# tenstack/batch-scheduler

Measured on AMD Instinct MI355X. Metric: pod x node fit evals/sec, higher is better.
Workload: dtype int64; 1 GPU; cfg3/tail: 10000 pods / 2000 groups / 5000 nodes, 5 int64 lanes (cpu, mem, eph, pods, gpu), seed 20260921; stages=prefilter+filter+tally+ready, parallelism=single GPU

## Files before the change

batch-scheduler_amd/csrc/bs_fast.hpp:

```cpp
#pragma once

#include "bs_kernels.hpp"
#include "bs_filter_t.hpp"

#ifdef BS_NT_TABLES
#define BS_TBL_STORE(p, v) __builtin_nontemporal_store((v), (p))
#else
#define BS_TBL_STORE(p, v) (*(p) = (v))
#endif
namespace bs {

template <bool INL = false>
__device__ __forceinline__ void arm_tally(const GroupsDev& gr, const BatchDev& b, const BatchParams& prm, uint32_t i, uint32_t nthreads);

__device__ __forceinline__ const uint8_t* range_glocal(const BatchDev& b) { return reinterpret_cast<const uint8_t*>(b.pod_ranges); }
__device__ __forceinline__ const uint32_t* range_start(const BatchDev& b, uint32_t G) { return b.pod_ranges + (G + 3u) / 4u; }
__device__ __forceinline__ const uint32_t* range_lfirst(const BatchDev& b, uint32_t G, uint32_t pod_blocks) { return range_start(b, G) + pod_blocks + 1u; }
__device__ __forceinline__ bool range_local_on(const BatchDev& b, const BatchParams& prm) {
  return b.pod_ranges && prm.do_tally && prm.do_ready && !prm.filter_deny;
}

#if BS_EMIT_MAIN
__global__ void k_pods_prep(unsigned long long* tables, uint32_t ntab, uint32_t* gstat, uint32_t ngstat, uint32_t* kcount, uint32_t* gcount, uint32_t G) {
  const uint32_t t = blockIdx.x * blockDim.x + threadIdx.x, nt = gridDim.x * blockDim.x;
// ... 263 lines not shown
    for (uint32_t j = 0; j < BS_MAX_LANES; ++j)
      if (j < sh.L()) times.v[j] = wmul(lp.mr.v[j], not_finished);
    times.present = lp.mr.present;
    res_add(out, times, sh, gate);
  }
  if (out.v[BS_LANE_PODS] == 0) out.v[BS_LANE_PODS] = mm + 1;
}
template <int TS>
__device__ __forceinline__ uint32_t filter_slot_values(const Res& cur_in, const LeaderPre& lp, Shape<TS> sh, uint32_t gate, int64_t (&R)[4], int64_t (&M)[4]) {
  Res ms, cur = cur_in;
  res_zero(ms, sh);
  res_add(ms, lp.mr, sh, gate);
  res_add(cur, ms, sh, gate);
  uint32_t ff = 0;
#pragma unroll
  for (uint32_t s = 0; s < BS_MAX_SCALARS; ++s) {
    if (s < sh.S()) {
      if ((cur.present & (1u << s)) && cur.v[4 + s] != 0) ff |= 1u;
      if ((ms.present & (1u << s)) && ms.v[4 + s] != 0) ff |= 2u;
    }
  }
#pragma unroll
  for (int j = 0; j < 4; ++j) { R[j] = cur.v[j]; M[j] = ms.v[j]; }
  return ff;
}
template <int TS, bool PUB = false>
__device__ __forceinline__ void filter_slot_from(const BatchDev& b, const BatchParams& prm, const Res& cur_in, const LeaderPre& lp, Shape<TS> sh, uint32_t gate,
                                                 uint32_t slot, bool zero_feas = true) {
  if (!lp.have_mr) return;
  int64_t R[4], M[4];
  const uint32_t ff = filter_slot_values(cur_in, lp, sh, gate, R, M);
  if (zero_feas) st_pub<PUB>(&b.fu_feas[slot], 0u);
  int64_t* dst2 = b.uparams + (size_t)slot * 8;
#pragma unroll
  for (int j = 0; j < 4; ++j) { st_pub<PUB>(&dst2[j], R[j]); st_pub<PUB>(&dst2[4 + j], M[j]); }
  st_pub<PUB>(&b.uflags[slot], ff | ((uint32_t)BS_FL_EVALUATED << 8) | (prm.stamp << 16));
}
template <int TS>
__device__ __forceinline__ uint32_t class_scan_query(const Res& cur, const LeaderPre& lp0, Shape<TS> sh, uint32_t gate, Res& q) {
  pre_allocated_from(lp0, sh, gate, q);
  res_add(q, cur, sh, gate);
  uint32_t absok = 0;
#pragma unroll
  for (uint32_t s2 = 0; s2 < BS_MAX_SCALARS; ++s2) {
    if (s2 < sh.S()) {
      const bool pres = q.present & (1u << s2);
      if (!pres || q.v[4 + s2] == 0) absok |= 1u << s2;
      if (!pres) q.v[4 + s2] = INT64_MIN;
    }
  }
  return q.present | (absok << 16);
}

template <int TS, bool PUB = false, bool SLOTS = true, bool INL = false>
__device__ __forceinline__ void fast_query_thread(const PodsDev& pods, const GroupsDev& gr, const BatchDev& b, const BatchParams& prm, uint32_t i,
                                                  uint32_t nthreads, uint32_t end = BS_INF, uint32_t t = BS_INF) {
  const Shape<TS> sh(prm.S);
  const bool valid = i < pods.p && i < end;
  const uint32_t gate = prm.eph_gate;
  const uint32_t ii = valid ? i : 0u;
  const int32_t leader0 = b.leader_epoch[0];
  const uint8_t panic0 = b.panic_epoch[0];
  const uint32_t K = prm.run_filter ? (prm.k_host ? prm.k_host : *b.kclass) : 0u;
  const int32_t gi = pods.p ? pods.group[ii] : BS_POD_NOT_GROUPED;
  const uint8_t pfl = pods.p ? pods.flags[ii] : (uint8_t)0;
  const uint64_t own = pods.p ? pods.owner[ii] : 0ull;
  const uint32_t pc = pods.p ? b.pclass[ii] : 0u;
  const uint32_t pp = pods.p ? b.ppair[ii] : BS_INF;
  Res cur;
  if (pods.p) pod_require(pods, ii, sh, gate, cur); else res_zero(cur, sh);
  arm_tally<INL>(gr, b, prm, t == BS_INF ? i : t, nthreads);
  if (i < 8 && prm.collect_stats) b.stats[i] = 0;
  const bool grouped = valid && gi >= 0 && (uint32_t)gi < gr.g;
  const uint32_t g = grouped ? (uint32_t)gi : 0u;
  const uint8_t gfl = gr.g ? gr.flags[g] : (uint8_t)0;
  const uint64_t occ0 = gr.g ? gr.occupied[g] : 0ull;
  const uint32_t fo = gr.g ? b.first_owner_s[g] : BS_INF;
  const uint32_t anchor = grouped ? b.first_pod_s[g] : i;
  LeaderPre lp0{}, lp1{};
  const bool two = prm.run_filter && prm.sop_leader0 >= 0 && prm.sop_leader0 != leader0;
  if (gr.g) {
    leader_pre_load(gr, leader0, sh, lp0);
    if (two) leader_pre_load(gr, prm.sop_leader0, sh, lp1); else lp1 = lp0;
  }
  const bool need_fo = grouped && occ0 == 0 && fo != BS_INF && i > fo;
  const uint64_t occ_fo = need_fo ? pods.owner[fo] : 0ull;
  const uint32_t owner_rank = valid ? owner_rank_of(b, prm, anchor, pods.p) : 0u;

  uint8_t code = BS_PF_PASS_NOT_GROUPED, st = 0;
  bool has_q = false;
  Res q;
  res_zero(q, sh);
  if (valid) {
    if (owner_rank == prm.rank) st |= ST_OWNED;
    if (gi == BS_POD_NOT_GROUPED) code = BS_PF_PASS_NOT_GROUPED;
    else if (pfl & BS_POD_LAST_PERMITTED) code = BS_PF_PASS_LAST_PERMITTED;
    else if (!grouped) code = BS_PF_ERR_PG_NOT_FOUND;
    else if ((gfl & BS_GROUP_DENIED) || fd_denied(b, (uint32_t)gi, i)) code = BS_PF_ERR_DENIED;
    else {
      st |= ST_ELIG;
      bool occ_err = false;
      if (occ0 != 0) occ_err = (own == 0) || (own != occ0);
      else if (need_fo) occ_err = (own == 0) || (own != occ_fo);
      if (occ_err) code = BS_PF_ERR_OCCUPIED;
      else if (panic0) code = BS_PF_PANIC_DIV0;
      else {
        st |= ST_REACH6;
        if (leader0 < 0) code = BS_PF_PASS_NO_MAX;
        else if (leader0 == gi) code = BS_PF_PASS_IS_MAX;
        else {
          pre_allocated_from(lp0, sh, gate, q);
          res_add(q, cur, sh, gate);
          code = BS_PF_PASS_RESERVE_FITS;
          has_q = (st & ST_OWNED) != 0;
        }
      }
    }
    if (has_q) st |= ST_QUERY;
    b.tcode[i] = code;
    b.stage[i] = st;
  }
  BS_STAMP(1, 1);
  {
    __shared__ uint32_t s_reach;
    if (threadIdx.x == 0) s_reach = BS_INF;
    __syncthreads();
    const unsigned long long rb = __ballot(valid && (st & ST_REACH6));
    if (rb && lane_id() == __ffsll((long long)rb) - 1) atomicMin(&s_reach, i);
    __syncthreads();
    if (threadIdx.x == 0) st_pub<INL>(&b.first_reach64[blockIdx.x], ((unsigned long long)prm.seq_inv << 32) | s_reach);
  }
  BS_STAMP(1, 2);
  const uint32_t qslot = has_q ? pc : 0u;
  bool fill = SLOTS && wave_elect_by_key(qslot, has_q);
  bool w1 = false, w2 = false;
  if (SLOTS && prm.run_filter) {
    const bool may = valid && (st & ST_OWNED) && BS_PF_IS_PASS(code) && grouped;
    w1 = wave_elect_by_key(pc, may && leader0 >= 0 && leader0 != gi);
    w2 = wave_elect_by_key(pc, may && prm.sop_leader0 >= 0 && prm.sop_leader0 != gi);
  }
  if constexpr (PUB) {
    uint32_t o1 = 0, o2 = 0, o3 = 0;
    if (w1) o1 = __hip_atomic_exchange(&b.uclaim[pc], prm.stamp, __ATOMIC_RELAXED, __HIP_MEMORY_SCOPE_AGENT);
    if (w2) o2 = __hip_atomic_exchange(&b.uclaim[pc + K], prm.stamp, __ATOMIC_RELAXED, __HIP_MEMORY_SCOPE_AGENT);
    if (fill) o3 = __hip_atomic_exchange(&b.qstamp_s[qslot], prm.stamp, __ATOMIC_RELAXED, __HIP_MEMORY_SCOPE_AGENT);
    if (w1 && o1 == prm.stamp) w1 = false;
    if (w2 && o2 == prm.stamp) w2 = false;
    if (fill && o3 == prm.stamp) fill = false;
  }
  if (w1) filter_slot_from<TS, PUB>(b, prm, cur, lp0, sh, gate, pc);
  if (w2) filter_slot_from<TS, PUB>(b, prm, cur, lp1, sh, gate, pc + K);
  BS_STAMP(1, 3);
  if (has_q) {
    b.qpos[i] = qslot;
    atomicMin(&b.pair_firstq[pp], ((unsigned long long)prm.seq_inv << 32) | i);
  }
  if (fill) {
    uint32_t absok = 0;
#pragma unroll
    for (uint32_t s = 0; s < BS_MAX_SCALARS; ++s) {
      if (s < sh.S()) {
        const bool pres = q.present & (1u << s);
        if (!pres || q.v[4 + s] == 0) absok |= 1u << s;
        if (!pres) q.v[4 + s] = INT64_MIN;
      }
    }
    const uint32_t slot = qslot;
    int64_t* dst = b.qreq_s + (size_t)slot * prm.LP;
#pragma unroll
    for (uint32_t j = 0; j < BS_MAX_LANES; ++j)
      if (j < prm.LP) st_pub<PUB>(&dst[j], j < sh.L() ? q.v[j] : (int64_t)INT64_MIN);
    st_pub<PUB>(&b.qflags_s[slot], q.present | (absok << 16));
    st_pub<PUB>(&b.qtab_s[slot], (int32_t)0);
    st_pub<PUB>(&b.first_row[slot], BS_INF);
// ... 32 lines not shown
    Res ms;
    res_zero(ms, sh);
    if (have && lp.have_mr) res_add(ms, lp.mr, sh, gate);
    uint32_t ff = (have && lp.have_mr) ? 1u : 0u;
#pragma unroll
    for (uint32_t q = 0; q < BS_MAX_SCALARS; ++q)
      if (q < sh.S() && (ms.present & (1u << q)) && ms.v[4 + q] != 0) ff |= 2u;
    const unsigned long long holds = __ballot(l[0] >= ms.v[0] && l[1] >= ms.v[1] && l[2] >= ms.v[2] && l[3] >= ms.v[3]);
    if (stores) {
      b.nodew[nodew_pair(stride, s, w)] = ok;
      b.nodew[nodew_pair(stride, s, w) + 1] = ~holds;
    }
    if (blk == 0 && threadIdx.x == 0) {
#pragma unroll
      for (int j = 0; j < 4; ++j) b.nodew[nodew_ref_lane(stride, s, j)] = (uint64_t)ms.v[j];
      b.nodew[nodew_ref_flags(stride, s)] = ff;
    }
  }
}

template <int TS>
__global__ __launch_bounds__(kTblChunk) void k_fast_query_tables(PodsDev pods, GroupsDev gr, NodesDev nd, BatchDev b, BatchDev bt, BatchParams prm,
                                                                 const TableDesc* forced, uint32_t nchunks, uint32_t query_blocks) {
  BS_STAMP(1, 0);
  if (blockIdx.x < query_blocks) fast_query_thread<TS>(pods, gr, b, prm, blockIdx.x * kTblChunk + threadIdx.x, query_blocks * kTblChunk);
  else if (blockIdx.x < query_blocks + nchunks) tables_local_fast<TS>(nd, bt, prm, forced, blockIdx.x - query_blocks);
  else node_words_block<TS>(gr, nd, b, prm, blockIdx.x - query_blocks - nchunks);
  BS_STAMP(1, 7);
}

template <int NL>
__device__ __forceinline__ unsigned long long rows_cover(unsigned long long m, const int64_t (&a)[BS_MAX_LANES], const int64_t (&r)[BS_MAX_LANES]) {
  asm volatile("s_mov_b64 exec, %[m]\n\tv_cmpx_ge_i64 vcc, %[a0], %[r0]\n\tv_cmpx_ge_i64 vcc, %[a1], %[r1]\n\tv_cmpx_ge_i64 vcc, %[a2], %[r2]\n\t"
               "v_cmpx_ge_i64 vcc, %[a3], %[r3]\n\ts_mov_b64 %[m], exec\n\ts_mov_b64 exec, -1"
               : [m] "+s"(m)
               : [a0] "v"(a[0]), [r0] "v"(r[0]), [a1] "v"(a[1]), [r1] "v"(r[1]), [a2] "v"(a[2]), [r2] "v"(r[2]), [a3] "v"(a[3]), [r3] "v"(r[3])
               : "vcc");
#pragma unroll
  for (int j = 4; j < NL; ++j)
    asm volatile("s_mov_b64 exec, %[m]\n\tv_cmpx_ge_i64 vcc, %[a], %[r]\n\ts_mov_b64 %[m], exec\n\ts_mov_b64 exec, -1" : [m] "+s"(m) : [a] "v"(a[j]), [r] "v"(r[j]) : "vcc");
  return m;
}
#ifndef BS_SCAN_BALLOT
#define BS_SCAN_BALLOT 1
#endif
constexpr uint32_t kSpinBound = 1u << 18;
__device__ __forceinline__ void test_chaos_delay() {
#ifdef BS_TEST_CHAOS
  uint32_t h = (blockIdx.x + 1u) * 2654435761u ^ (uint32_t)wall_clock64() * 40503u;
  h ^= h >> 15; h *= 2246822519u; h ^= h >> 13;
  for (uint32_t s = 0; s < (h & 15u); ++s) __builtin_amdgcn_s_sleep(127);
#endif
}
constexpr uint32_t kStepSlotsMax = 256;
__device__ __forceinline__ bool step_wait(const uint32_t* word, uint32_t base, uint32_t need, int32_t* h_err) {
  uint32_t spins = 0;
  while ((uint32_t)(ld_agent(word) - base) < need) {
    __builtin_amdgcn_s_sleep(1);
    if (++spins > kSpinBound) { if (h_err) __hip_atomic_store(h_err, 1, __ATOMIC_RELAXED, __HIP_MEMORY_SCOPE_SYSTEM); return false; }
  }
  return true;
}
constexpr uint32_t kScanRecChunks = 64;
constexpr uint32_t kFeasRecGroups = 32;
#ifndef BS_GATHER_DIRECT
#define BS_GATHER_DIRECT 8
#endif
constexpr uint32_t kGatherDirectBlocks = BS_GATHER_DIRECT;
constexpr uint32_t kRecStride = 32;
constexpr uint32_t kTkSlots = 32, kTkTab = 48, kTkP1 = 64, kTkDone = 64 + 16 * 16, kTkWays = 16, kTkWords = 64 + 2 * 16 * 16;
__device__ __forceinline__ void spread_add(uint32_t* words, uint32_t who) {
  (void)__hip_atomic_fetch_add(&words[16u * (who % kTkWays)], 1u, __ATOMIC_RELAXED, __HIP_MEMORY_SCOPE_AGENT);
}
__device__ __forceinline__ bool spread_wait(const uint32_t* words, uint32_t base, uint32_t need, int32_t* h_err) {
  uint32_t spins = 0;
  for (;;) {
    uint32_t v = lane_id() < (int)kTkWays ? ld_agent(&words[16u * (uint32_t)lane_id()]) : 0u;
#pragma unroll
    for (int o = 1; o < (int)kTkWays; o <<= 1) v += (uint32_t)__shfl_xor((int)v, o);
    v = (uint32_t)__builtin_amdgcn_readfirstlane((int)v);
    if ((uint32_t)(v - base) >= need) return true;
    __builtin_amdgcn_s_sleep(4);
    if (++spins > kSpinBound) { if (h_err && lane_id() == 0) __hip_atomic_store(h_err, 1, __ATOMIC_RELAXED, __HIP_MEMORY_SCOPE_SYSTEM); return false; }
  }
}
template <int TS, bool REGS = false>
__device__ __forceinline__ void table_scan_block(const NodesDev& nd, const BatchDev& b, const BatchParams& prm, const TableDesc* forced, uint32_t chunk, uint32_t nchunks,
                                                 uint32_t share, uint32_t nshares, uint32_t pod_blocks, uint32_t tk_pods0, uint32_t tk_tab0, const GroupsDev& gr,
                                                 const int64_t* ckeys, const uint32_t* cpres, uint32_t kcap, bool direct = false, uint32_t forced_cls = 0) {
  __shared__ unsigned long long s_wtot[BS_MAX_LANES][4];
  __shared__ uint32_t s_kp[BS_MAX_SCALARS];
  __shared__ unsigned long long s_off[BS_MAX_LANES];
  __shared__ uint32_t s_kpg[BS_MAX_SCALARS];
  __shared__ int64_t s_req[kStepSlotsMax][BS_MAX_LANES];
  __shared__ uint32_t s_qf[kStepSlotsMax];
  __shared__ uint32_t s_first[kStepSlotsMax];
  BS_STAMP(2, 0);
  const Shape<TS> sh(prm.S);
  const uint32_t L = sh.L(), S = sh.S(), LP = prm.LP;
  const uint32_t k = chunk * kTblChunk + threadIdx.x;
  const bool in_range = REGS ? k < nd.n : k < nd.m;
  const uint32_t n = REGS ? (in_range ? k : 0u) : (in_range ? nd.kmap[k] : 0u);
  const TableDesc d = REGS ? TableDesc{forced_cls, 0.7f} : *forced;
  const uint32_t fw = nd.fit[(size_t)d.cls * nd.fit_words + (n >> 5)];
  const uint8_t fl = nd.flags[n];
  const bool valid = in_range && (!REGS || !(fl & BS_NODE_SKIP_MASK));
  const uint32_t ap = nd.apres[n], rp = nd.rpres[n];
  int64_t al[BS_MAX_LANES], rq[BS_MAX_LANES];
#pragma unroll
  for (uint32_t j = 0; j < BS_MAX_LANES; ++j) {
    if (j < L) {
      al[j] = nd.alloc[(size_t)j * nd.stride + n];
      rq[j] = nd.req[(size_t)j * nd.stride + n];
    }
  }
  const uint32_t K = prm.k_host ? prm.k_host : *b.kclass;
  const uint32_t per = (K + nshares - 1u) / nshares, s_lo = share * per, s_hi = min(K, s_lo + per);
  Res raw;
  int32_t leader0 = -1;
  uint8_t panic0 = 0;
  LeaderPre lp0{};
  if constexpr (REGS) {
    const uint32_t cc = s_lo + threadIdx.x < s_hi ? s_lo + threadIdx.x : 0u;
#pragma unroll
    for (uint32_t j = 0; j < BS_MAX_LANES; ++j)
      if (j < L) raw.v[j] = ckeys[(size_t)j * kcap + cc];
    raw.present = cpres[cc];
    leader0 = b.leader_epoch[0];
    panic0 = b.panic_epoch[0];
    if (gr.g) leader_pre_load(gr, leader0, sh, lp0);
  }
  const bool fit = valid && ((fw >> (n & 31u)) & 1u) && !(fl & BS_NODE_TAINT_ERR);
  const uint32_t pres = fit ? (ap & rp) : 0u;
  if (threadIdx.x < BS_MAX_SCALARS) s_kp[threadIdx.x] = BS_INF;
  for (uint32_t t = threadIdx.x; t < kStepSlotsMax; t += kTblChunk) s_first[t] = BS_INF;
  unsigned long long incl[BS_MAX_LANES];
  const int w = wave_id();
#pragma unroll
  for (uint32_t j = 0; j < BS_MAX_LANES; ++j) {
    incl[j] = 0;
    if (j < L) {
      const bool live = fit && (j < 4 || (pres & (1u << (j - 4)))) && !(j == BS_LANE_EPH && !prm.eph_gate);
      const unsigned long long left = live ? (unsigned long long)wsub(scale_f32(al[j], d.pct), rq[j]) : 0ull;
      incl[j] = wave_incl_scan_add_u64(left);
      if (lane_id() == 63) s_wtot[j][w] = incl[j];
    }
  }
  __syncthreads();
#pragma unroll
// ... 365 lines not shown
  if (threadIdx.x == 0) {
    __hip_atomic_store(&b.ticket[0], 0u, __ATOMIC_RELAXED, __HIP_MEMORY_SCOPE_AGENT);
    if constexpr (WT && BS_HOME_WT) __hip_atomic_store(b.h_tag, prm.host_tag, __ATOMIC_RELAXED, __HIP_MEMORY_SCOPE_SYSTEM);
    else __hip_atomic_store(b.h_tag, prm.host_tag, __ATOMIC_RELEASE, __HIP_MEMORY_SCOPE_SYSTEM);
  }
}

__device__ __forceinline__ void tally_quorum_atomic(const BatchDev& b, const BatchParams& prm, bool grouped, uint32_t g, bool admit, uint32_t want, uint32_t ma,
                                                    uint32_t need) {
  unsigned long long mine = 0;
  bool asked = false;
  unsigned long long todo = __ballot(grouped);
  const unsigned long long adm = __ballot(grouped && admit);
  for (int round = 0; todo && round < kElectRounds; ++round) {
    const int leader = __ffsll((long long)todo) - 1;
    const uint32_t k0 = (uint32_t)__builtin_amdgcn_readlane((int)g, leader);
    const unsigned long long same = __ballot(grouped && g == k0) & todo;
    if (lane_id() == leader) {
      mine = ((unsigned long long)__popcll(same) << 32) | (unsigned long long)__popcll(same & adm);
      asked = true;
    }
    todo &= ~same;
  }
  if (todo & (1ull << lane_id())) {
    mine = (1ull << 32) | (admit ? 1ull : 0ull);
    asked = true;
  }
  unsigned long long got = 0;
  if (asked) got = __hip_atomic_fetch_add(&b.admit64[g], mine, __ATOMIC_RELAXED, __HIP_MEMORY_SCOPE_AGENT);
  if (asked) {
    const unsigned long long tot = got + mine;
    if ((uint32_t)(tot >> 32) == want) {
      const uint32_t ad = (uint32_t)tot;
      const uint8_t rd = (ma + ad) >= need ? 1 : 0;
      b.admit[g] = ad;
      b.ready[g] = rd;
      if (prm.host_tag) { st_home(&b.h_admit[g], ad); st_home(&b.h_ready[g], rd); }
    }
  }
}
template <bool WT = false>
__device__ __forceinline__ void tally_tail(const GroupsDev& gr, const BatchDev& b, const BatchParams& prm, bool grouped, uint32_t g, bool admit,
                                           uint32_t nblocks) {
  if (prm.do_tally && prm.do_ready) {
    uint32_t want = 0, ma = 0, mm = 0, sc = 0;
    if (grouped) { want = b.gcount[g]; ma = gr.matched[g]; mm = gr.min_member[g]; sc = gr.status_scheduled[g]; }
    tally_quorum_atomic(b, prm, grouped, g, admit, want, ma, (uint32_t)(mm - sc));
  } else if (prm.do_tally) {
    wave_aggregated_add(b.admit, g, grouped && admit);
  }
  final_tail<WT>(b, prm, nblocks);
}

constexpr uint32_t kLocalTag = 0x80000000u;
template <bool WT = false>
__device__ __forceinline__ void tally_tail_whole(const GroupsDev& gr, const BatchDev& b, const BatchParams& prm, bool grouped, uint32_t g, bool admit,
                                                 uint32_t nblocks, uint32_t gwant, uint32_t ma, uint32_t need, uint32_t* s_adm) {
  if (prm.do_tally && prm.do_ready) {
    const bool local = grouped && (gwant & kLocalTag);
    const uint32_t lslot = gwant & 0xFFu;
    if (local && admit) atomicAdd(&s_adm[lslot], 1u);
    __syncthreads();
    if (local && lslot == threadIdx.x) {
      const uint32_t ad = s_adm[lslot];
      const uint8_t rd = (ma + ad) >= need ? 1 : 0;
      b.admit[g] = ad;
      b.ready[g] = rd;
      if (prm.host_tag) { st_home(&b.h_admit[g], ad); st_home(&b.h_ready[g], rd); }
    }
    tally_quorum_atomic(b, prm, grouped && !local, g, admit, gwant, ma, need);
  } else if (prm.do_tally) {
    wave_aggregated_add(b.admit, g, grouped && admit);
  }
  final_tail<WT>(b, prm, nblocks);
}


template <bool INL = false>
__device__ __forceinline__ void fast_final_block(const PodsDev& pods, const GroupsDev& gr, const NodesDev& nd, const BatchDev& b, const BatchParams& prm,
                                                 uint32_t query_blocks, uint32_t bx, uint32_t nblocks, uint32_t producers, uint32_t tk_p1 = 0, uint32_t aux = 0,
                                                 uint32_t tk_done = 0, uint32_t hint_blocks = 0, uint32_t p0 = BS_INF, uint32_t p1 = BS_INF) {
  __shared__ uint32_t s_first_reach;
  __shared__ uint32_t s_rowk[INL ? kStepSlotsMax : 1u], s_feask[INL ? 2u * kStepSlotsMax : 1u], s_ladm[INL ? 256u : 1u], s_gw[INL ? 3u : 1u][INL ? 256u : 1u];
  BS_STAMP(3, 0);
  if constexpr (INL) {
    s_ladm[threadIdx.x] = 0u;
    if (threadIdx.x < 64) (void)spread_wait(&b.ticket[kTkP1], tk_p1, query_blocks, b.h_err);
    __syncthreads();
  }
  const uint32_t dx = bx * 256u + threadIdx.x;
  const uint32_t i = p0 == BS_INF ? dx : p0 + threadIdx.x;
  const bool valid = i < pods.p && (p0 == BS_INF || i < p1);
  uint8_t code0 = 0, st0 = 0;
  int32_t gi0 = BS_POD_NOT_GROUPED;
  uint32_t qpos0 = 0, pclass0 = 0, pair0 = BS_INF;
  uint32_t lfirst = BS_INF;
  if (valid) { code0 = b.tcode[i]; st0 = b.stage[i]; gi0 = pods.group[i]; qpos0 = b.qpos[i]; pclass0 = b.pclass[i]; pair0 = b.ppair[i]; }
  if (INL && valid && range_local_on(b, prm)) lfirst = range_lfirst(b, gr.g, query_blocks)[i];
  const uint32_t K = prm.k_host ? prm.k_host : *b.kclass;
  const int32_t leader_now = b.leader_epoch[0];
  if (threadIdx.x < 64) {
    uint32_t found = BS_INF;
    for (uint32_t b0 = 0; b0 < query_blocks && found == BS_INF; b0 += 64u) {
      const uint32_t bk = b0 + threadIdx.x;
      uint32_t v = BS_INF;
      if (bk < query_blocks) {
        const unsigned long long w = INL ? ld_agent64(&b.first_reach64[bk]) : b.first_reach64[bk];
        if ((uint32_t)(w >> 32) == prm.seq_inv) v = (uint32_t)w;
      }
      const unsigned long long any = __ballot(v != BS_INF);
      if (any) found = (uint32_t)__shfl((int)v, __ffsll((long long)any) - 1);
    }
    if (threadIdx.x == 0) s_first_reach = found;
  }
  const bool owned = valid && (st0 & ST_OWNED);
  const bool walk = owned && (st0 & ST_ELIG);
  const bool grouped = valid && gi0 >= 0 && (uint32_t)gi0 < gr.g;
  uint32_t row_q = BS_INF, row_c = BS_INF, feas0 = 0, feas1 = 0;
  unsigned long long head = ~0ull, own_fq = ~0ull, own_next = ~0ull;
  if (walk) {
    head = b.pair_head[gi0];
    if (pair0 != BS_INF) { own_fq = INL ? ld_agent64(&b.pair_firstq[pair0]) : b.pair_firstq[pair0]; own_next = b.pair_next[pair0]; }
  }
  if constexpr (INL) {
    if (prm.do_tally && prm.do_ready) {
      uint32_t gwant = 0, gma = 0, gneed = 0;
      if (grouped) {
        gma = gr.matched[gi0];
        gneed = (uint32_t)(gr.min_member[gi0] - gr.status_scheduled[gi0]);
        gwant = lfirst != BS_INF ? kLocalTag | (lfirst - p0) : b.gcount[gi0];
      }
      s_gw[0][threadIdx.x] = gwant;
      s_gw[1][threadIdx.x] = gma;
      s_gw[2][threadIdx.x] = gneed;
    }
  }
  if (producers) {
    asm volatile("s_waitcnt vmcnt(0)" ::: "memory");
    if constexpr (INL) {
      const uint32_t tagw = prm.seq_inv, U = prm.run_filter ? 2u * K : 0u;
      uint32_t groups = 0;
      if (prm.run_filter) {
        uint32_t tiles, bpw, nchunk;
        step_filter_split(K, (nd.n + 63u) / 64u, aux, tiles, bpw, nchunk);
        groups = (nchunk + 3u) / 4u;
      }
      const unsigned long long none = ((unsigned long long)tagw << 32) | BS_INF, zero = (unsigned long long)tagw << 32;
      BS_STAMP(3, 4);
      if (query_blocks > kGatherDirectBlocks) {
        if (threadIdx.x < 64) (void)spread_wait(&b.ticket[kTkDone], tk_done, hint_blocks, b.h_err);
      } else
      for (uint32_t spins = 0;; ++spins) {
        uint32_t andt = tagw, ort = tagw, row = BS_INF, fs[2] = {0u, 0u};
        if (threadIdx.x < K) {
          const unsigned long long* rec = b.scan_rec + threadIdx.x;
          for (uint32_t c0 = 0; c0 < producers; c0 += 8u) {
            unsigned long long w[8];
#pragma unroll
            for (uint32_t u = 0; u < 8u; ++u) w[u] = c0 + u < producers ? ld_agent64(&rec[(size_t)(c0 + u) * kStepSlotsMax]) : none;
#pragma unroll
            for (uint32_t u = 0; u < 8u; ++u) { andt &= (uint32_t)(w[u] >> 32); ort |= (uint32_t)(w[u] >> 32); row = min(row, (uint32_t)w[u]); }
          }
        }
#pragma unroll
        for (uint32_t h = 0; h < 2u; ++h) {
          const uint32_t slot = threadIdx.x + 256u * h;
          if (slot < U) {
            const unsigned long long* rec = b.feas_rec + slot;
            for (uint32_t g0 = 0; g0 < groups; g0 += 8u) {
              unsigned long long w[8];
#pragma unroll
              for (uint32_t u = 0; u < 8u; ++u) w[u] = g0 + u < groups ? ld_agent64(&rec[(size_t)(g0 + u) * (2u * kStepSlotsMax)]) : zero;
#pragma unroll
              for (uint32_t u = 0; u < 8u; ++u) { andt &= (uint32_t)(w[u] >> 32); ort |= (uint32_t)(w[u] >> 32); fs[h] += (uint32_t)w[u]; }
            }
          }
        }
        const bool timed_out = spins > kSpinBound / 2u;
        if (__syncthreads_and((andt == tagw && ort == tagw) || timed_out)) {
          if (threadIdx.x < K) s_rowk[threadIdx.x] = row;
#pragma unroll
          for (uint32_t h = 0; h < 2u; ++h)
            if (threadIdx.x + 256u * h < U) s_feask[threadIdx.x + 256u * h] = fs[h];
          if (timed_out && threadIdx.x == 0 && b.h_err) __hip_atomic_store(b.h_err, 1, __ATOMIC_RELAXED, __HIP_MEMORY_SCOPE_SYSTEM);
          BS_COUNT(3, 5, spins + 1u);
          break;
        }
        __builtin_amdgcn_s_sleep(2);
// ... 45 lines not shown
          }
        }
        denied = fr < i;
        if (prm.commit && fr == i) b.fast_reject[gi] = fr;
      }
      if (denied) code = BS_PF_ERR_DENIED;
      else if (st & ST_QUERY) {
        if (row_q == BS_INF) { code = BS_PF_REJECT_RESERVE; fk = BS_K_NONE; }
        else fk = INL ? row_q : nd.kmap[row_q];
      }
    } else {
      code = BS_PF_NOT_OWNED;
    }
    b.pf_code[i] = code;
    b.pf_first_k[i] = fk;
    const bool reached = i >= first_reach;
    const int32_t leader = reached ? leader_now : prm.sop_leader0;
    b.pf_leader[i] = leader;
    if (prm.host_tag) { st_home(&b.h_pf_code[i], code); st_home(&b.h_pf_first_k[i], fk); st_home(&b.h_pf_leader[i], leader); }
    const bool pass = code != BS_PF_NOT_OWNED && BS_PF_IS_PASS(code);
    uint32_t feasible = 1u, slot = 0;
    uint8_t fl = BS_FL_NOT_RUN;
    if (prm.run_filter) {
      if (pass) {
        if (gi == BS_POD_NOT_GROUPED) fl = BS_FL_PASS_NOT_GROUPED;
        else if (gi < 0 || (uint32_t)gi >= gr.g) fl = BS_FL_ERR_PG_NOT_FOUND;
        else if (leader < 0) fl = BS_FL_PANIC_NIL_MAX;
        else if (leader == gi) fl = BS_FL_PASS_IS_MAX;
        else { fl = BS_FL_EVALUATED; slot = pclass0 + (reached ? 0u : K); }
      }
      feasible = fl == BS_FL_EVALUATED ? (reached ? feas0 : feas1) : (fl < 16u ? nd.n : 0u);
      b.fu_slot[i] = slot;
      b.fl_feasible[i] = feasible;
    } else {
      b.fl_feasible[i] = 0;
    }
    b.fl_code[i] = fl;
    b.fflags[i] = (uint32_t)fl << 8;
    if (prm.host_tag) { st_home(&b.h_fl_code[i], fl); st_home(&b.h_fl_feasible[i], prm.run_filter ? feasible : 0u); st_home(&b.h_fl_slot[i], slot); }
    if (gi >= 0 && (uint32_t)gi < gr.g && pass && feasible > 0) admit = true;
    if (prm.filter_deny && fl == BS_FL_EVALUATED && feasible < nd.n) atomicMin(&b.fd_event[gi], ((unsigned long long)prm.seq_inv << 32) | i);
  }
  if (gathered) {
    if (prm.run_filter)
      for (uint32_t k = dx; k < 2u * K; k += nblocks * 256u) b.fu_feas[k] = s_feask[INL ? k : 0u];
  }
  if (prm.host_tag && prm.run_filter) {
    const uint32_t U = min(2u * K, b.hstride);
    for (uint32_t k = dx; k < U; k += nblocks * 256u) st_home(&b.h_feas[k], gathered ? s_feask[INL ? k : 0u] : ld_agent(&b.fu_feas[k]));
  }
  BS_STAMP(3, 2);
  if (!prm.filter_deny) {
    if constexpr (INL)
      tally_tail_whole<true>(gr, b, prm, grouped, grouped ? (uint32_t)gi0 : 0u, admit, nblocks, s_gw[0][threadIdx.x], s_gw[1][threadIdx.x], s_gw[2][threadIdx.x], s_ladm);
    else
      tally_tail<true>(gr, b, prm, grouped, grouped ? (uint32_t)gi0 : 0u, admit, nblocks);
  }
  BS_STAMP(3, 7);
}

template <int S>
__global__ __launch_bounds__(256) void k_fast_scan_filter(PodsDev pods, NodesDev nd, BatchDev bt, BatchParams prm, uint32_t m, uint32_t jcap,
                                                          uint32_t scan_blocks, uint32_t filter_waves, uint32_t ustride) {
  __shared__ int64_t s_rows[4][64][4 + S];
  if (blockIdx.x < scan_blocks)
    scan_loop<S, true, 1>(bt, prm, m, jcap, 0u, 0u, 1u, blockIdx.x, scan_blocks, s_rows[wave_id()]);
  else
    filter_loop<2>(pods, nd, bt, filter_waves, 1u, ustride, prm.collect_stats, blockIdx.x - scan_blocks, gridDim.x - scan_blocks, prm.stamp, 2u * prm.k_host);
}
template <int S>
__global__ __launch_bounds__(256) void k_fast_scan(BatchDev bt, BatchParams prm, uint32_t m, uint32_t jcap) {
  __shared__ int64_t s_rows[4][64][4 + S];
  scan_loop<S, true, 1>(bt, prm, m, jcap, 0u, 0u, 1u, blockIdx.x, gridDim.x, s_rows[wave_id()]);
}
template <int PU, bool DB>
__global__ __launch_bounds__(256) void k_fast_filter(PodsDev pods, NodesDev nd, BatchDev bt, BatchParams prm, uint32_t filter_waves, uint32_t ustride) {
  filter_loop<2, PU, DB>(pods, nd, bt, filter_waves, 1u, ustride, prm.collect_stats, blockIdx.x, gridDim.x, prm.stamp, 2u * prm.k_host);
}
#if BS_EMIT_FAST
__global__ __launch_bounds__(256) __attribute__((amdgpu_waves_per_eu(7))) void k_fast_filter_w7(PodsDev pods, NodesDev nd, BatchDev bt, BatchParams prm, uint32_t filter_waves,
                                                                                                uint32_t ustride) {
  filter_loop<2, 2, false>(pods, nd, bt, filter_waves, 1u, ustride, prm.collect_stats, blockIdx.x, gridDim.x, prm.stamp, 2u * prm.k_host);
}
#endif
#if BS_EMIT_FAST
__global__ __launch_bounds__(256) void k_fast_filter_t(NodesDev nd, BatchDev bt, BatchParams prm, uint32_t filter_waves, uint32_t ustride, uint32_t by_tile) {
  filter_loop_t<false>(nd, bt, filter_waves, ustride, prm.collect_stats, blockIdx.x, gridDim.x, prm.stamp, 2u * prm.k_host, by_tile);
}
#endif
template <int S>
__global__ __launch_bounds__(256) __attribute__((amdgpu_waves_per_eu(S <= 1 ? 4 : 1))) void k_fast_scan_filter_t(NodesDev nd, BatchDev bt, BatchParams prm, uint32_t m, uint32_t jcap, uint32_t scan_blocks,
                                                            uint32_t filter_waves, uint32_t ustride, uint32_t form) {
  __shared__ int64_t s_rows[4][64][4 + S];
  const uint32_t filter_first = form & 1u, by_tile = form & 2u;
  const uint32_t filter_blocks = gridDim.x - scan_blocks;
  const bool is_scan = filter_first ? blockIdx.x >= filter_blocks : blockIdx.x < scan_blocks;
  BS_STAMP(2, 0);
  if (is_scan)
    scan_loop<S, true, 1>(bt, prm, m, jcap, 0u, 0u, 1u, filter_first ? blockIdx.x - filter_blocks : blockIdx.x, scan_blocks, s_rows[wave_id()]);
  else
    filter_loop_t<true>(nd, bt, filter_waves, ustride, prm.collect_stats, filter_first ? blockIdx.x : blockIdx.x - scan_blocks, filter_blocks, prm.stamp, 2u * prm.k_host, by_tile);
  BS_STAMP(2, 7);
}
#if BS_EMIT_MAIN
__global__ __launch_bounds__(256) void k_fast_final(PodsDev pods, GroupsDev gr, NodesDev nd, BatchDev b, BatchParams prm, uint32_t query_blocks) {
  fast_final_block(pods, gr, nd, b, prm, query_blocks, blockIdx.x, gridDim.x, 0u);
}
#endif

template <int S>
__global__ __launch_bounds__(256) void k_fast_scan_filter_final(PodsDev pods, GroupsDev gr, NodesDev nd, BatchDev b, BatchDev bt, BatchParams prm, uint32_t m,
                                                                uint32_t jcap, uint32_t scan_blocks, uint32_t filter_blocks, uint32_t filter_waves,
                                                                uint32_t ustride, uint32_t query_blocks) {
  __shared__ int64_t s_rows[4][64][4 + S];
  const uint32_t producers = scan_blocks + filter_blocks;
  test_chaos_delay();
#ifdef BS_TEST_LATE_ROLE_B
  {
    const int role = blockIdx.x < scan_blocks ? 0 : blockIdx.x < producers ? 1 : 2;
    if (role == BS_TEST_LATE_ROLE_B) for (int spin = 0; spin < 20; ++spin) __builtin_amdgcn_s_sleep(127);
  }
#endif
  if (blockIdx.x < producers) {
    BS_STAMP(2, 0);
    if (blockIdx.x < scan_blocks)
      scan_loop<S, true, 2>(bt, prm, m, jcap, 0u, 0u, 1u, blockIdx.x, scan_blocks, s_rows[wave_id()]);
    else
      filter_loop<2>(pods, nd, bt, filter_waves, 1u, ustride, prm.collect_stats, blockIdx.x - scan_blocks, filter_blocks, prm.stamp, 2u * prm.k_host);
    asm volatile("s_waitcnt vmcnt(0)" ::: "memory");
    __syncthreads();
    if (threadIdx.x == 0) (void)__hip_atomic_fetch_add(&b.ticket[1], 1u, __ATOMIC_RELAXED, __HIP_MEMORY_SCOPE_AGENT);
    BS_STAMP(2, 7);
    return;
  }
  fast_final_block(pods, gr, nd, b, prm, query_blocks, blockIdx.x - producers, gridDim.x - producers, producers);
}

template <int TS, bool WHOLE>
__global__ __launch_bounds__(kTblChunk) void k_fast_step_a(PodsDev pods, GroupsDev gr, NodesDev nd, BatchDev b, BatchDev bt, BatchParams prm, const TableDesc* forced,
                                                           uint32_t nchunks, uint32_t query_blocks, uint32_t nshares, uint32_t filter_blocks, uint32_t filter_waves,
                                                           uint32_t ustride, uint32_t tk_pods0, uint32_t tk_tab0, uint32_t param_blocks, const int64_t* ckeys,
                                                           const uint32_t* cpres, uint32_t kcap, uint32_t tk_p1, uint32_t tk_done, uint32_t forced_cls) {
  BS_STAMP(1, 0);
  test_chaos_delay();
  const uint32_t tb = nchunks * nshares;
#ifdef BS_TEST_LATE_ROLE
  {
    const int role = blockIdx.x < query_blocks ? 0 : blockIdx.x < query_blocks + param_blocks ? 1 : blockIdx.x < query_blocks + param_blocks + tb ? 2 : 3;
    if (role == BS_TEST_LATE_ROLE) for (int spin = 0; spin < 20; ++spin) __builtin_amdgcn_s_sleep(127);
  }
#endif
  const uint32_t producers = param_blocks ? param_blocks : query_blocks;
  const bool direct = query_blocks <= kGatherDirectBlocks;
  if (blockIdx.x < query_blocks) {
    if constexpr (WHOLE) {
      const uint32_t p0 = b.pod_ranges ? range_start(b, gr.g)[blockIdx.x] : blockIdx.x * kTblChunk;
      const uint32_t p1 = b.pod_ranges ? range_start(b, gr.g)[blockIdx.x + 1u] : pods.p;
      fast_query_thread<TS, false, false, true>(pods, gr, b, prm, p0 + threadIdx.x, query_blocks * kTblChunk, p1, blockIdx.x * kTblChunk + threadIdx.x);
      asm volatile("s_waitcnt vmcnt(0)" ::: "memory");
      __syncthreads();
      if (threadIdx.x == 0) spread_add(&b.ticket[kTkP1], blockIdx.x);
      fast_final_block<true>(pods, gr, nd, b, prm, query_blocks, blockIdx.x, query_blocks, nchunks, tk_p1, filter_waves, tk_done, tb + filter_blocks, p0, p1);
    } else if (param_blocks) {
      fast_query_thread<TS, false, false>(pods, gr, b, prm, blockIdx.x * kTblChunk + threadIdx.x, query_blocks * kTblChunk);
    } else {
      fast_query_thread<TS, true>(pods, gr, b, prm, blockIdx.x * kTblChunk + threadIdx.x, query_blocks * kTblChunk);
      BS_STAMP(1, 4);
      asm volatile("s_waitcnt vmcnt(0)" ::: "memory");
      __syncthreads();
      BS_STAMP(1, 5);
      if (threadIdx.x == 0) (void)__hip_atomic_fetch_add(&b.ticket[kTkSlots], 1u, __ATOMIC_RELAXED, __HIP_MEMORY_SCOPE_AGENT);
    }
  } else if (blockIdx.x < query_blocks + param_blocks) {
    class_slots_block<TS>(gr, b, prm, ckeys, cpres, kcap, blockIdx.x - query_blocks, !(WHOLE && direct));
  } else if (blockIdx.x < query_blocks + param_blocks + tb) {
    const uint32_t x = blockIdx.x - query_blocks - param_blocks;
    table_scan_block<TS, WHOLE>(nd, bt, prm, forced, x / nshares, nchunks, x % nshares, nshares, producers, tk_pods0, tk_tab0, gr, ckeys, cpres, kcap, direct, forced_cls);
    if constexpr (WHOLE) {
      if (!direct) {
        asm volatile("s_waitcnt vmcnt(0)" ::: "memory");
        __syncthreads();
        if (threadIdx.x == 0) spread_add(&b.ticket[kTkDone], blockIdx.x);
      }
    }
  } else if constexpr (WHOLE) {
    step_filter_block<TS>(gr, nd, bt, prm, ckeys, cpres, kcap, filter_waves, ustride, blockIdx.x - query_blocks - param_blocks - tb, filter_blocks, direct, tk_pods0, producers);
    if (!direct) {
      asm volatile("s_waitcnt vmcnt(0)" ::: "memory");
      __syncthreads();
      if (threadIdx.x == 0) spread_add(&b.ticket[kTkDone], blockIdx.x);
    }
  } else {
    __shared__ uint32_t s_go;
    if (threadIdx.x == 0) {
      s_go = step_wait(&b.ticket[kTkSlots], tk_pods0, producers, b.h_err) ? 1u : 0u;
      __builtin_amdgcn_fence(__ATOMIC_ACQUIRE, "agent");
    }
    __syncthreads();
    if (!s_go) return;
    filter_loop<2>(pods, nd, bt, filter_waves, 1u, ustride, prm.collect_stats, blockIdx.x - query_blocks - param_blocks - tb, filter_blocks, prm.stamp, 2u * prm.k_host);
  }
  BS_STAMP(1, 7);
}


template <int TS>
__global__ __launch_bounds__(kTblChunk) void k_tables_local_nofix(NodesDev nd, BatchDev b, BatchParams prm, uint32_t nchunks, uint32_t cstride,
                                                                  uint32_t gstride) {
  const uint32_t slot = blockIdx.x;
  if (!b.needed[slot]) return;
  BatchDev bt = b;
  bt.tables = b.tables + (size_t)slot * prm.mcap * prm.LP;
  bt.kp = b.kp + (size_t)slot * 16;
  bt.chunk_tot = b.chunk_tot + (size_t)slot * cstride * 16;
  bt.chunk_kp = b.chunk_kp + (size_t)slot * cstride * 16;
  bt.gmax = b.gmax + (size_t)slot * gstride * prm.LP;
  const TableDesc d = table_desc(slot, prm.C, nullptr);
  tables_local_fast<TS>(nd, bt, prm, &d, blockIdx.y);
}

#if BS_EMIT_MAIN
__global__ __launch_bounds__(kLeaderBlock) void k_leader_scan(GroupsDev gr, BatchDev b) {
  __shared__ unsigned long long s_w[kLeaderBlock / 64];
  __shared__ uint32_t s_p[kLeaderBlock / 64];
  __shared__ unsigned long long s_carry;
  __shared__ uint32_t s_pcarry, s_nexact, s_exact[64];
  const uint32_t E1 = *b.nepochs;
  auto key_of = [&](uint32_t g, bool& panic) -> unsigned long long {
    if (gr.flags[g] & BS_GROUP_SCHEDULED_LATCH) return 0ull;
    const uint32_t f = leader_finished(gr, g, panic);
// ... 85 lines not shown
```

Before: 3713 billion evals/s.

## Share LDS arena across block roles and hand pod state to final block via LDS

Introduces a single shared-memory arena in the fused step kernel, used by the table-scan role and the whole-pod query/final role, so the kernel's LDS footprint is the max rather than the sum of both roles. The query phase writes per-pod code, stage, group, class and pair into LDS so the final block reads them locally instead of reloading tcode/stage/group/pclass/ppair from global memory. Group metadata (pair_head, pair_next, matched, min_member, status, gcount) loads are moved before the ticket spin-wait to overlap their latency with waiting. Risk: qpos is replaced by pclass in the inline path, and the early global loads assume the data are stable before the wait.

```diff
diff --git a/batch-scheduler_amd/csrc/bs_fast.hpp b/batch-scheduler_amd/csrc/bs_fast.hpp
--- a/batch-scheduler_amd/csrc/bs_fast.hpp
+++ b/batch-scheduler_amd/csrc/bs_fast.hpp
@@ -339,9 +339,39 @@
   return q.present | (absok << 16);
 }
 
+constexpr uint32_t kStepSlotsMax = 256;
+struct PodLds {
+  uint32_t* rowk;
+  uint32_t* feask;
+  uint32_t* ladm;
+  uint32_t* gw;
+  uint32_t* pk;
+  uint32_t* gi;
+  uint32_t* pc;
+  uint32_t* pair;
+};
+constexpr uint32_t kPodRec = 1u << 31;
+constexpr uint32_t kLocalTag = 0x80000000u;
+constexpr uint32_t kArenaTableBytes = kStepSlotsMax * BS_MAX_LANES * 8u + 2u * kStepSlotsMax * 4u;
+constexpr uint32_t kArenaPodBytes = (3u * kStepSlotsMax + 256u + 3u * 256u + 4u * 256u) * 4u;
+constexpr uint32_t kStepArenaBytes = kArenaTableBytes > kArenaPodBytes ? kArenaTableBytes : kArenaPodBytes;
+__device__ __forceinline__ PodLds pod_lds(unsigned char* arena) {
+  uint32_t* w = reinterpret_cast<uint32_t*>(arena);
+  PodLds o;
+  o.rowk = w; w += kStepSlotsMax;
+  o.feask = w; w += 2u * kStepSlotsMax;
+  o.ladm = w; w += 256u;
+  o.gw = w; w += 3u * 256u;
+  o.pk = w; w += 256u;
+  o.gi = w; w += 256u;
+  o.pc = w; w += 256u;
+  o.pair = w;
+  return o;
+}
+
 template <int TS, bool PUB = false, bool SLOTS = true, bool INL = false>
 __device__ __forceinline__ void fast_query_thread(const PodsDev& pods, const GroupsDev& gr, const BatchDev& b, const BatchParams& prm, uint32_t i,
-                                                  uint32_t nthreads, uint32_t end = BS_INF, uint32_t t = BS_INF) {
+                                                  uint32_t nthreads, uint32_t end = BS_INF, uint32_t t = BS_INF, const PodLds* pl = nullptr) {
   const Shape<TS> sh(prm.S);
   const bool valid = i < pods.p && i < end;
   const uint32_t gate = prm.eph_gate;
@@ -407,6 +437,13 @@
     b.tcode[i] = code;
     b.stage[i] = st;
   }
+  if constexpr (INL) {
+    const uint32_t x = threadIdx.x;
+    pl->pk[x] = valid ? (kPodRec | (uint32_t)code | ((uint32_t)st << 8)) : 0u;
+    pl->gi[x] = valid ? (uint32_t)gi : (uint32_t)BS_POD_NOT_GROUPED;
+    pl->pc[x] = valid ? pc : 0u;
+    pl->pair[x] = valid ? pp : BS_INF;
+  }
   BS_STAMP(1, 1);
   {
     __shared__ uint32_t s_reach;
@@ -545,7 +582,6 @@
   for (uint32_t s = 0; s < (h & 15u); ++s) __builtin_amdgcn_s_sleep(127);
 #endif
 }
-constexpr uint32_t kStepSlotsMax = 256;
 __device__ __forceinline__ bool step_wait(const uint32_t* word, uint32_t base, uint32_t need, int32_t* h_err) {
   uint32_t spins = 0;
   while ((uint32_t)(ld_agent(word) - base) < need) {
@@ -580,14 +616,15 @@
 template <int TS, bool REGS = false>
 __device__ __forceinline__ void table_scan_block(const NodesDev& nd, const BatchDev& b, const BatchParams& prm, const TableDesc* forced, uint32_t chunk, uint32_t nchunks,
                                                  uint32_t share, uint32_t nshares, uint32_t pod_blocks, uint32_t tk_pods0, uint32_t tk_tab0, const GroupsDev& gr,
-                                                 const int64_t* ckeys, const uint32_t* cpres, uint32_t kcap, bool direct = false, uint32_t forced_cls = 0) {
+                                                 const int64_t* ckeys, const uint32_t* cpres, uint32_t kcap, unsigned char* arena, bool direct = false,
+                                                 uint32_t forced_cls = 0) {
   __shared__ unsigned long long s_wtot[BS_MAX_LANES][4];
   __shared__ uint32_t s_kp[BS_MAX_SCALARS];
   __shared__ unsigned long long s_off[BS_MAX_LANES];
   __shared__ uint32_t s_kpg[BS_MAX_SCALARS];
-  __shared__ int64_t s_req[kStepSlotsMax][BS_MAX_LANES];
-  __shared__ uint32_t s_qf[kStepSlotsMax];
-  __shared__ uint32_t s_first[kStepSlotsMax];
+  int64_t (*s_req)[BS_MAX_LANES] = reinterpret_cast<int64_t (*)[BS_MAX_LANES]>(arena);
+  uint32_t* s_qf = reinterpret_cast<uint32_t*>(arena + kStepSlotsMax * BS_MAX_LANES * 8u);
+  uint32_t* s_first = s_qf + kStepSlotsMax;
   BS_STAMP(2, 0);
   const Shape<TS> sh(prm.S);
   const uint32_t L = sh.L(), S = sh.S(), LP = prm.LP;
@@ -1059,7 +1096,6 @@
   final_tail<WT>(b, prm, nblocks);
 }
 
-constexpr uint32_t kLocalTag = 0x80000000u;
 template <bool WT = false>
 __device__ __forceinline__ void tally_tail_whole(const GroupsDev& gr, const BatchDev& b, const BatchParams& prm, bool grouped, uint32_t g, bool admit,
                                                  uint32_t nblocks, uint32_t gwant, uint32_t ma, uint32_t need, uint32_t* s_adm) {
@@ -1086,24 +1122,48 @@
 template <bool INL = false>
 __device__ __forceinline__ void fast_final_block(const PodsDev& pods, const GroupsDev& gr, const NodesDev& nd, const BatchDev& b, const BatchParams& prm,
                                                  uint32_t query_blocks, uint32_t bx, uint32_t nblocks, uint32_t producers, uint32_t tk_p1 = 0, uint32_t aux = 0,
-                                                 uint32_t tk_done = 0, uint32_t hint_blocks = 0, uint32_t p0 = BS_INF, uint32_t p1 = BS_INF) {
+                                                 uint32_t tk_done = 0, uint32_t hint_blocks = 0, uint32_t p0 = BS_INF, uint32_t p1 = BS_INF,
+                                                 unsigned char* arena = nullptr) {
   __shared__ uint32_t s_first_reach;
-  __shared__ uint32_t s_rowk[INL ? kStepSlotsMax : 1u], s_feask[INL ? 2u * kStepSlotsMax : 1u], s_ladm[INL ? 256u : 1u], s_gw[INL ? 3u : 1u][INL ? 256u : 1u];
+  PodLds L{};
+  if constexpr (INL) L = pod_lds(arena);
+  uint32_t* const s_rowk = L.rowk;
+  uint32_t* const s_feask = L.feask;
+  uint32_t* const s_ladm = L.ladm;
   BS_STAMP(3, 0);
-  if constexpr (INL) {
-    s_ladm[threadIdx.x] = 0u;
-    if (threadIdx.x < 64) (void)spread_wait(&b.ticket[kTkP1], tk_p1, query_blocks, b.h_err);
-    __syncthreads();
-  }
   const uint32_t dx = bx * 256u + threadIdx.x;
   const uint32_t i = p0 == BS_INF ? dx : p0 + threadIdx.x;
   const bool valid = i < pods.p && (p0 == BS_INF || i < p1);
   uint8_t code0 = 0, st0 = 0;
   int32_t gi0 = BS_POD_NOT_GROUPED;
   uint32_t qpos0 = 0, pclass0 = 0, pair0 = BS_INF;
-  uint32_t lfirst = BS_INF;
-  if (valid) { code0 = b.tcode[i]; st0 = b.stage[i]; gi0 = pods.group[i]; qpos0 = b.qpos[i]; pclass0 = b.pclass[i]; pair0 = b.ppair[i]; }
-  if (INL && valid && range_local_on(b, prm)) lfirst = range_lfirst(b, gr.g, query_blocks)[i];
+  unsigned long long head = ~0ull, own_fq = ~0ull, own_next = ~0ull;
+  if constexpr (INL) {
+    const uint32_t x = threadIdx.x, pk = L.pk[x];
+    code0 = (uint8_t)pk;
+    st0 = (uint8_t)(pk >> 8);
+    gi0 = (int32_t)L.gi[x];
+    pclass0 = L.pc[x];
+    qpos0 = pclass0;
+    pair0 = L.pair[x];
+    const bool grp = valid && gi0 >= 0 && (uint32_t)gi0 < gr.g;
+    uint32_t lfirst = BS_INF, gwant = 0, gma = 0, gmm = 0, gsc = 0;
+    if (valid && range_local_on(b, prm)) lfirst = range_lfirst(b, gr.g, query_blocks)[i];
+    if (grp) {
+      head = b.pair_head[gi0];
+      if (pair0 != BS_INF) own_next = b.pair_next[pair0];
+      if (prm.do_tally && prm.do_ready) { gma = gr.matched[gi0]; gmm = gr.min_member[gi0]; gsc = gr.status_scheduled[gi0]; gwant = b.gcount[gi0]; }
+    }
+    s_ladm[x] = 0u;
+    if (x < 64) (void)spread_wait(&b.ticket[kTkP1], tk_p1, query_blocks, b.h_err);
+    __syncthreads();
+    if (grp && prm.do_tally && prm.do_ready && lfirst != BS_INF) gwant = kLocalTag | (lfirst - p0);
+    L.gw[x] = gwant;
+    L.gw[256u + x] = gma;
+    L.gw[512u + x] = (uint32_t)(gmm - gsc);
+  } else if (valid) {
+    code0 = b.tcode[i]; st0 = b.stage[i]; gi0 = pods.group[i]; qpos0 = b.qpos[i]; pclass0 = b.pclass[i]; pair0 = b.ppair[i];
+  }
   const uint32_t K = prm.k_host ? prm.k_host : *b.kclass;
   const int32_t leader_now = b.leader_epoch[0];
   if (threadIdx.x < 64) {
@@ -1124,23 +1184,11 @@
   const bool walk = owned && (st0 & ST_ELIG);
   const bool grouped = valid && gi0 >= 0 && (uint32_t)gi0 < gr.g;
   uint32_t row_q = BS_INF, row_c = BS_INF, feas0 = 0, feas1 = 0;
-  unsigned long long head = ~0ull, own_fq = ~0ull, own_next = ~0ull;
-  if (walk) {
+  if constexpr (INL) {
+    if (walk && pair0 != BS_INF) own_fq = ld_agent64(&b.pair_firstq[pair0]);
+  } else if (walk) {
     head = b.pair_head[gi0];
-    if (pair0 != BS_INF) { own_fq = INL ? ld_agent64(&b.pair_firstq[pair0]) : b.pair_firstq[pair0]; own_next = b.pair_next[pair0]; }
-  }
-  if constexpr (INL) {
-    if (prm.do_tally && prm.do_ready) {
-      uint32_t gwant = 0, gma = 0, gneed = 0;
-      if (grouped) {
-        gma = gr.matched[gi0];
-        gneed = (uint32_t)(gr.min_member[gi0] - gr.status_scheduled[gi0]);
-        gwant = lfirst != BS_INF ? kLocalTag | (lfirst - p0) : b.gcount[gi0];
-      }
-      s_gw[0][threadIdx.x] = gwant;
-      s_gw[1][threadIdx.x] = gma;
-      s_gw[2][threadIdx.x] = gneed;
-    }
+    if (pair0 != BS_INF) { own_fq = b.pair_firstq[pair0]; own_next = b.pair_next[pair0]; }
   }
   if (producers) {
     asm volatile("s_waitcnt vmcnt(0)" ::: "memory");
@@ -1292,7 +1340,7 @@
   BS_STAMP(3, 2);
   if (!prm.filter_deny) {
     if constexpr (INL)
-      tally_tail_whole<true>(gr, b, prm, grouped, grouped ? (uint32_t)gi0 : 0u, admit, nblocks, s_gw[0][threadIdx.x], s_gw[1][threadIdx.x], s_gw[2][threadIdx.x], s_ladm);
+      tally_tail_whole<true>(gr, b, prm, grouped, grouped ? (uint32_t)gi0 : 0u, admit, nblocks, L.gw[threadIdx.x], L.gw[256u + threadIdx.x], L.gw[512u + threadIdx.x], s_ladm);
     else
       tally_tail<true>(gr, b, prm, grouped, grouped ? (uint32_t)gi0 : 0u, admit, nblocks);
   }
@@ -1383,6 +1431,7 @@
                                                            const uint32_t* cpres, uint32_t kcap, uint32_t tk_p1, uint32_t tk_done, uint32_t forced_cls) {
   BS_STAMP(1, 0);
   test_chaos_delay();
+  __shared__ __align__(16) unsigned char s_arena[kStepArenaBytes];
   const uint32_t tb = nchunks * nshares;
 #ifdef BS_TEST_LATE_ROLE
   {
@@ -1396,11 +1445,12 @@
     if constexpr (WHOLE) {
       const uint32_t p0 = b.pod_ranges ? range_start(b, gr.g)[blockIdx.x] : blockIdx.x * kTblChunk;
       const uint32_t p1 = b.pod_ranges ? range_start(b, gr.g)[blockIdx.x + 1u] : pods.p;
-      fast_query_thread<TS, false, false, true>(pods, gr, b, prm, p0 + threadIdx.x, query_blocks * kTblChunk, p1, blockIdx.x * kTblChunk + threadIdx.x);
+      const PodLds pl = pod_lds(s_arena);
+      fast_query_thread<TS, false, false, true>(pods, gr, b, prm, p0 + threadIdx.x, query_blocks * kTblChunk, p1, blockIdx.x * kTblChunk + threadIdx.x, &pl);
       asm volatile("s_waitcnt vmcnt(0)" ::: "memory");
       __syncthreads();
       if (threadIdx.x == 0) spread_add(&b.ticket[kTkP1], blockIdx.x);
-      fast_final_block<true>(pods, gr, nd, b, prm, query_blocks, blockIdx.x, query_blocks, nchunks, tk_p1, filter_waves, tk_done, tb + filter_blocks, p0, p1);
+      fast_final_block<true>(pods, gr, nd, b, prm, query_blocks, blockIdx.x, query_blocks, nchunks, tk_p1, filter_waves, tk_done, tb + filter_blocks, p0, p1, s_arena);
     } else if (param_blocks) {
       fast_query_thread<TS, false, false>(pods, gr, b, prm, blockIdx.x * kTblChunk + threadIdx.x, query_blocks * kTblChunk);
     } else {
@@ -1415,7 +1465,8 @@
     class_slots_block<TS>(gr, b, prm, ckeys, cpres, kcap, blockIdx.x - query_blocks, !(WHOLE && direct));
   } else if (blockIdx.x < query_blocks + param_blocks + tb) {
     const uint32_t x = blockIdx.x - query_blocks - param_blocks;
-    table_scan_block<TS, WHOLE>(nd, bt, prm, forced, x / nshares, nchunks, x % nshares, nshares, producers, tk_pods0, tk_tab0, gr, ckeys, cpres, kcap, direct, forced_cls);
+    table_scan_block<TS, WHOLE>(nd, bt, prm, forced, x / nshares, nchunks, x % nshares, nshares, producers, tk_pods0, tk_tab0, gr, ckeys, cpres, kcap, s_arena, direct,
+                                forced_cls);
     if constexpr (WHOLE) {
       if (!direct) {
         asm volatile("s_waitcnt vmcnt(0)" ::: "memory");
```

Measured after the change: 3772 billion evals/s, median of 5. 1.02x the previous value.
